# OrangeSodahub/InfGen

Measured on AMD Instinct MI355X. Metric: agent-steps/sec (closed-loop rollout), higher is better.
Workload: dtype f32

## Files before the change

### include/infgen_hip.h

```cpp
#ifndef INFGEN_HIP_H_
#define INFGEN_HIP_H_

#include <stdint.h>

#ifdef __cplusplus
extern "C" {
#endif

#define INFGEN_MAX_LAYERS 8

enum {
  INFGEN_Q_ATTN_PACK_SIZE = 0,
  INFGEN_Q_FOURIER_PACK_SIZE_N2 = 1,
  INFGEN_Q_FOURIER_PACK_SIZE_N3 = 2,
  INFGEN_Q_FOURIER_PACK_SIZE_N4 = 3,
  INFGEN_Q_TILE_ROWS = 4,
  INFGEN_Q_EDGE_ATTN_CAP = 5,
  INFGEN_Q_MAX_AGENTS = 6,
  INFGEN_Q_ABI_VERSION = 7,
  INFGEN_Q_SIZEOF_ROLLOUT = 8,
  INFGEN_Q_ATTN_SPLIT_ROWS = 9,
  INFGEN_Q_HEADS_SAMPLE_K = 10,
};
int infgen_layout_query(int what);
// ... 103 lines not shown
                    float* Q, float* U, float* K, float* V, void* stream);
int infgen_edge_attn(int rows, const float* Q, const float* U, const float* Ksrc, const float* Vsrc,
                     const int* off, const int* cnt, const int* src, const float* rhat,
                     float* AGG, float* Z, float* SIG, void* stream);
int infgen_edge_attn_fused(int rows, const float* Q, const float* pack, const float* Ksrc, const float* Vsrc,
                           const int* off, const int* cnt, const int* src, const float* rhat,
                           float* AGG, void* stream);
int infgen_fourier_embed_r24(const float* raw, int n_dims, const int* count_dev, int e_cap, const float* pack, void* out, void* stream);
int infgen_edge_attn_fused_r24(int rows, const float* Q, const float* pack, const float* Ksrc, const float* Vsrc,
                               const int* off, const int* cnt, const int* src, const void* rhat24, float* AGG, void* stream);
int infgen_set_rhat_format(int format);
int infgen_set_edge_kernel(int kernel);
int infgen_set_edge_fuse(int mode);
int infgen_get_options(InfgenOptions* out);
int infgen_thread_options(const InfgenOptions* o);
int infgen_get_effective_options(InfgenOptions* out);
int infgen_edge_fused_occupancy(void);
int infgen_debug_stream_read(const float* p, unsigned long long n_bytes, int width, float* out, void* stream);
int infgen_set_edge_loop(int variant);
int infgen_set_overlap(int mode);
int infgen_set_layers_p(int mode);
int infgen_layers_p_capacity(void);
int infgen_edge_attn_mode(int rows, const float* Q, const float* U, const float* Ksrc, const float* Vsrc,
                          const int* off, const int* cnt, const int* src, const float* rhat,
                          float* AGG, float* Z, float* SIG, int wide, void* stream);
int infgen_attn_post(float* X, int rows, const float* pack, const float* AGG, const float* Z, const float* SIG,
                     int has_pos, void* stream);
int infgen_attn_post_pre(float* X, int rows, const float* pack, const float* AGG, const float* Z, const float* SIG,
                         int has_pos, const float* next_pack, float* nQ, float* nU, float* nK, float* nV, void* stream);
int infgen_heads(const float* X, int rows, const float* tok_pack, const float* st_pack, int token_size,
                 float* logits, int* next_token, int* next_state, void* stream);
int infgen_heads_logprob(const float* X, int rows, const float* tok_pack, const float* st_pack, int token_size,
                         float* logits, int* next_token, int* next_state, float* token_logprob, void* stream);
int infgen_token_logprob(const float* logits, int rows, int n, const int* token, float* out, void* stream);
int infgen_heads_sample(const float* X, int rows, const float* tok_pack, const float* st_pack, int token_size, int k,
                        const float* uniform, float* logits, int* next_token, int* next_state, float* token_logprob,
                        float* sample_logprob, void* stream);
int infgen_heads_sample_ex(const float* X, int rows, const float* tok_pack, const float* st_pack, int token_size, int k,
                           const float* uniform, const InfgenSampling* sampling, float* logits, int* next_token, int* next_state,
                           float* token_logprob, float* sample_logprob, void* stream);
int infgen_heads_sample_mask(const float* X, int rows, const float* tok_pack, const float* st_pack, int token_size, int k,
                             const float* uniform, const InfgenSampling* sampling, const uint32_t* mask_bits, int mask_n_sets,
                             const int* mask_row, const int* mask_type, const int* type, float* logits,
                             int* next_token, int* next_state, float* token_logprob, float* sample_logprob, void* stream);
int infgen_heads_sample_fused(int attn_mode, int rows, int k);
int infgen_heads_logprob_fused(int attn_mode, int rows);
int infgen_map_token_head(const float* X, int ldx, const int* gather, int n, const float* pack, int token_size,
                          float* hidden, float* logits, long long* top_idx, void* stream);
int infgen_embedding_sum4(const float* tab0, const long long* idx0, int n0, const float* tab1, const long long* idx1, int n1,
                          const float* tab2, const long long* idx2, int n2, const float* tab3, const long long* idx3, int n3,
                          int rows, float* out, void* stream);
int infgen_map_graph(int S, int M_cap, const int* n_map, const float* pos, const float* orient, float radius,
                     int max_nbr, int* off, int* cnt, int* src, float* raw, int* total, int cap, void* stream);

int infgen_rollout_validate(const InfgenRollout* r);
int infgen_build_edges(const InfgenRollout* r, int c, int edgeless, void* stream);
int infgen_integrate(const InfgenRollout* r, int t, void* stream);
int infgen_raw_feature(const InfgenRollout* r, int col, void* stream);
int infgen_raw_feature_rows(const InfgenRollout* r, int col, const int* row_list, const int* row_mask, int n, void* stream);
int infgen_decode_layers(const InfgenRollout* r, int c, int edgeless, void* stream);
int infgen_decode_step(const InfgenRollout* r, int t, void* stream);
int infgen_rollout_run(const InfgenRollout* r, int t0, int t1, void* stream);
int infgen_command_rows(const InfgenRollout* r, int t, int kind, const int* cmd_token, const float* cmd_pose,
                        const unsigned char* cmd_mask, const float* shape, float* cmd_cost, void* stream);

int infgen_branch_scenes(const InfgenRollout* r, int t, const int* parent, int* n_bad, void* stream);
int infgen_resample_parents(const int* ancestor, int S0, int copies, int* parent, void* stream);

int infgen_snapshot_bytes(const InfgenRollout* r, int t, long long* bytes);
int infgen_snapshot_scenes(const InfgenRollout* r, int t, const int* slots, int n, void* snap, long long entry_stride, int* head,
                           int* n_bad, void* stream);
int infgen_restore_scenes(const InfgenRollout* r, int t, const int* index, const void* snap, long long entry_stride, const int* head,
                          int n, int* n_bad, void* stream);

int infgen_sample_topk(const float* logits, int rows, int n, int k, const float* uniform, int* token, void* stream);
int infgen_sample_topk_logprob(const float* logits, int rows, int n, int k, const float* uniform, int* token,
                               float* sample_logprob, void* stream);
int infgen_sample_topk_ex(const float* logits, int rows, int n, int k, const float* uniform, const InfgenSampling* sampling,
                          int* token, float* sample_logprob, int* nucleus, void* stream);
int infgen_sample_topk_mask(const float* logits, int rows, int n, int k, const float* uniform, const InfgenSampling* sampling,
                            const uint32_t* mask_bits, int mask_n_sets, const int* mask_row, const int* mask_type, const int* type,
                            int* token, float* sample_logprob, int* nucleus, void* stream);
int infgen_token_mask_create(const uint32_t* mask_bits, int mask_n_sets, const int* mask_row, const int* mask_type, const int* type);
int infgen_token_mask_destroy(int handle);

int infgen_collision_end_poses(const float* vocab, int token_size, float* end_pose, void* stream);
int infgen_collision_mask(const float* pos, const float* head, const int* state, const int* n_agents, const int* first_new,
                          const int* type, const float* shape, int S, int A_cap, int T, int c, const float* end_pose, int token_size,
                          int predict, float margin, const uint32_t* mask_bits, int mask_n_sets, const int* mask_row,
                          const int* mask_type, uint32_t* out_bits, int* out_count, void* stream);
int infgen_token_mask_collision(int handle, uint32_t* dyn_bits, const int* identity_row, const float* shape, const float* end_pose,
                                int predict, float margin, int* count);

int infgen_road_records_from_map(const float* map_pos, const float* map_orient, const long long* map_type, const long long* map_tok,
                                 const int* n_map, int S0, int M_cap, const float* map_vocab, int n_token, int detail, float* records,
                                 int rec_cap, int* n_records, void* stream);
int infgen_road_records_from_segments(const float* segments, const int* n_segments, int S0, int E, float* records, int rec_cap,
                                      int* n_records, void* stream);
int infgen_road_paths(const float* end_pose, int token_size, float* paths, void* stream);
int infgen_road_mask(const float* pos, const float* head, const int* state, const int* n_agents, const int* first_new, const int* type,
                     const float* shape, int S, int A_cap, int T, int c, const float* end_pose, const float* paths, int token_size,
                     const float* records, const int* n_records, int rec_cap, int copies, int sweep, float margin, const int* types,
                     const uint32_t* mask_bits, int mask_n_sets, const int* mask_row, const int* mask_type, uint32_t* out_bits,
                     int* out_count, void* stream);
int infgen_token_mask_road(int handle, uint32_t* road_bits, const int* identity_row, const float* shape, const float* end_pose,
                           const float* paths, const float* records, const int* n_records, int rec_cap, int copies, int sweep,
// ... 190 lines not shown
```

### infgen_amd/csrc/api.hip

```cpp
#include <cstdio>
#include <cstring>
#include <cstdlib>
#include <cmath>
#include <string>
#include <vector>
#include <atomic>
#include <mutex>
#include <unordered_map>
#include "kernels.h"
#include "../../include/infgen_hip.h"

using namespace ig;

static thread_local std::string g_err;

static int fail(const char* where, const char* what) {
  g_err = std::string(where) + ": " + what;
  return -1;
}
static int check_launch(const char* where) {
  hipError_t e = hipGetLastError();
  if (e != hipSuccess) return fail(where, hipGetErrorString(e));
  return 0;
}
// ... 651 lines not shown
}

extern "C" int infgen_edge_attn_fused(int rows, const float* Q, const float* pack, const float* Ksrc, const float* Vsrc,
                                      const int* off, const int* cnt, const int* src, const float* rhat,
                                      float* AGG, void* stream) {
  return edge_fused_launch(rows, Q, pack, Ksrc, Vsrc, EdgeSet{off, cnt, src, rhat}, AGG, 0, 0, stream);
}

extern "C" int infgen_fourier_embed_r24(const float* raw, int n, const int* count_dev, int e_cap, const float* pack, void* out,
                                        void* stream) {
  return fourier_embed_impl(raw, n, count_dev, e_cap, pack, nullptr, 0, static_cast<float*>(out), 128, 1, 1, stream);
}

extern "C" int infgen_edge_attn_fused_r24(int rows, const float* Q, const float* pack, const float* Ksrc, const float* Vsrc,
                                          const int* off, const int* cnt, const int* src, const void* rhat24,
                                          float* AGG, void* stream) {
  return edge_fused_launch(rows, Q, pack, Ksrc, Vsrc, EdgeSet{off, cnt, src, static_cast<const float*>(rhat24)}, AGG, 0, 0, stream, 1);
}

extern "C" int infgen_edge_attn(int rows, const float* Q, const float* U, const float* Ksrc, const float* Vsrc,
                                const int* off, const int* cnt, const int* src, const float* rhat,
                                float* AGG, float* Z, float* SIG, void* stream) {
  return edge_attn_impl(rows, Q, U, Ksrc, Vsrc, off, cnt, src, rhat, AGG, Z, SIG, rows <= 256 ? 1 : 0, stream);
}

extern "C" int infgen_edge_attn_mode(int rows, const float* Q, const float* U, const float* Ksrc, const float* Vsrc,
                                     const int* off, const int* cnt, const int* src, const float* rhat,
                                     float* AGG, float* Z, float* SIG, int wide, void* stream) {
  return edge_attn_impl(rows, Q, U, Ksrc, Vsrc, off, cnt, src, rhat, AGG, Z, SIG, wide, stream);
}

static int attn_post_fused(float* X, int rows, const float* pack, const float* AGG, const float* Z, const float* SIG,
                           int has_pos, const float* next_pack, float* nQ, float* nU, float* nK, float* nV, void* stream) {
  if (rows <= 0) return 0;
  { ProfScope _ps(INFGEN_KID_ATTN_POST, stream, attn_post_macs(rows, has_pos, next_pack, nQ, nU, nK, nV));
    if (attn_kind(rows)) {
      launch_attn_h(AttnHArgs{X, rows, pack, AGG, Z, SIG, has_pos, next_pack, 0, nQ, nU, nK, nV}, stream);
    } else {
      AttnPostArgs a{X, rows, pack, AGG, Z, SIG, has_pos, next_pack, nQ, nU, nK, nV};
      hipLaunchKernelGGL(k_attn_post, dim3(ceil_div(rows, TR)), dim3(NT), 0, (hipStream_t)stream, a);
    } }
  return check_launch("infgen_attn_post");
}

extern "C" int infgen_attn_post(float* X, int rows, const float* pack, const float* AGG, const float* Z,
                                const float* SIG, int has_pos, void* stream) {
  return attn_post_fused(X, rows, pack, AGG, Z, SIG, has_pos, nullptr, nullptr, nullptr, nullptr, nullptr, stream);
}

extern "C" int infgen_attn_post_pre(float* X, int rows, const float* pack, const float* AGG, const float* Z,
                                    const float* SIG, int has_pos, const float* next_pack, float* nQ, float* nU,
                                    float* nK, float* nV, void* stream) {
  return attn_post_fused(X, rows, pack, AGG, Z, SIG, has_pos, next_pack, nQ, nU, nK, nV, stream);
}

extern "C" int infgen_match_agent_tokens(const unsigned char* valid, const float* pos, const float* heading, const float* shape,
                                        const int* type, const float* tok, long long tok_agent_stride, int A, int T, int shift,
                                        int n_token, int* token_index, float* token_contour, void* stream) {
  if (A <= 0) return 0;
  if (shift <= 0 || T <= shift) return fail("infgen_match_agent_tokens", "need 0 < shift < T");
  if (n_token <= 0 || n_token > 2048) return fail("infgen_match_agent_tokens", "n_token must be in 1..2048");
  MatchTokensArgs a{valid, pos, heading, shape, type, tok, tok_agent_stride, A, T, shift, n_token, token_index, token_contour};
  hipLaunchKernelGGL(k_match_tokens, dim3(A), dim3(256), 0, (hipStream_t)stream, a);
  return check_launch("infgen_match_agent_tokens");
}

extern "C" int infgen_tokenize_agent(unsigned char* valid, float* pos, float* heading, float* velocity, const int* type,
                                    const float* tok, const float* shape_in, float* shape_out, float* wl_work, int A, int T,
                                    int shift, int current_step, int n_token, int invalid_state, int valid_state,
                                    int enter_state, int exit_state, int predict_state, int* token_index,
                                    float* token_contour, int* state_idx, float* token_pos, float* token_heading,
                                    unsigned char* token_valid, unsigned char* raw_token_valid, void* stream) {
  if (A <= 0) return 0;
  if (shift <= 0 || T <= shift || current_step < shift || current_step >= T)
    return fail("infgen_tokenize_agent", "need 0 < shift <= current_step < T");
  if (n_token <= 0 || n_token > 2048) return fail("infgen_tokenize_agent", "n_token must be in 1..2048");
  TokenizeArgs t{valid, pos, heading, velocity, type, wl_work, shape_in, shape_out, A, T, shift, current_step,
                 invalid_state, valid_state, enter_state, exit_state, predict_state, token_index, token_contour,
                 state_idx, token_pos, token_heading, token_valid, raw_token_valid};
  hipLaunchKernelGGL(k_tokenize_prep, dim3((A + 63) / 64), dim3(64), 0, (hipStream_t)stream, t);
  MatchTokensArgs m{valid, pos, heading, wl_work, type, tok, 0, A, T, shift, n_token, token_index, token_contour};
  hipLaunchKernelGGL(k_match_tokens, dim3(A), dim3(256), 0, (hipStream_t)stream, m);
  hipLaunchKernelGGL(k_tokenize_state, dim3((A + 63) / 64), dim3(64), 0, (hipStream_t)stream, t);
  return check_launch("infgen_tokenize_agent");
}

extern "C" int infgen_fetch_enterings(const float* token_pos, const float* token_heading, const int* state_idx,
                                     const int* agent_ptr, const int* av_index, int B, int max_agents, int T,
                                     const float* grid_xy, int grid_size, float radius, float angle_interval,
                                     int enter_state, int invalid_state, int* grid_token_idx, float* grid_offset_xy,
                                     int* heading_token_idx, int* sort_indices, unsigned char* inrange_mask,
                                     unsigned char* bos_mask, float* pos_xy, float* heading_theta, const float* pt_pos,
                                     int pt_stride, const int* pt_ptr, int M, int* pt_grid_token_idx, void* stream) {
  if (B <= 0 || T <= 0) return 0;
  if (max_agents > 2048) return fail("infgen_fetch_enterings", "more than 2048 agents in a scene");
  if (grid_size <= 0) return fail("infgen_fetch_enterings", "empty grid");
  EnteringsArgs a{token_pos, token_heading, state_idx, agent_ptr, av_index, B, T, grid_xy, grid_size, radius, angle_interval,
                  enter_state, invalid_state, grid_token_idx, grid_offset_xy, heading_token_idx, sort_indices, inrange_mask,
                  bos_mask, pos_xy, heading_theta, pt_pos, pt_stride, pt_ptr, M, pt_grid_token_idx};
  hipLaunchKernelGGL(k_fetch_enterings, dim3(B * T), dim3(256), 0, (hipStream_t)stream, a);
  if (pt_grid_token_idx && M > 0) {
    const long long waves = (long long)T * M;
    hipLaunchKernelGGL(k_pt_grid_cells, dim3((unsigned)((waves + 3) / 4)), dim3(256), 0, (hipStream_t)stream, a);
  }
  return check_launch("infgen_fetch_enterings");
}
// ... 1777 lines not shown
```

### infgen_amd/csrc/attn_h.hip

```cpp
#include <type_traits>
#include "kernels.h"
#include "layout.h"
#include "tile.cuh"
#include "split.cuh"
#include "attn_h.cuh"

namespace ig {

template <int WAVES, int TERMS>
__global__ __launch_bounds__(64 * WAVES, WAVES == 4 ? 2 : 1) void k_attn_h(AttnHArgs a) {
  constexpr int NTH = 64 * WAVES, TILE = 16 * WAVES;
  constexpr int XRING = WAVES == 4 ? IG_AH_RING4 : IG_AH_RING8;
  __shared__ __attribute__((aligned(16))) unsigned short Wb[XRING][QUARTER];
  __shared__ __attribute__((aligned(16))) float Vt[VT_SIZE];
  __shared__ const unsigned short* seg_ptr[5];
  __shared__ int seg_n[5];
  const int ngroups = a.groups ? *a.n_groups : (a.rows + 15) / 16;
  const int ntiles = (ngroups + WAVES - 1) / WAVES;
  if ((int)blockIdx.x >= ntiles) return;
  const int tid = threadIdx.x;
  const int lane = tid & 63, w = tid >> 6;
  const int j = lane & 15, rg = lane >> 4;
  const float* P = a.pack;
  const float* NP = a.next_pack;
// ... 181 lines not shown
        if (need_u) {
          u32x4 Qh[4], Ql[4];
          const float cq = frags_scaled(q, Qh, Ql) * hdr[1];
          float* urow = valid ? a.nU + (size_t)row * (H * D) : nullptr;
          for (int hp = 0; hp < 4; ++hp) {
            const unsigned short* Wl = take();
#pragma unroll
            for (int hh = 0; hh < 2; ++hh) {
              u32x2 qh, ql;
#define IG_PICK(S) case S: qh = hh ? u32x2{Qh[S][2], Qh[S][3]} : u32x2{Qh[S][0], Qh[S][1]}; \
                           ql = hh ? u32x2{Ql[S][2], Ql[S][3]} : u32x2{Ql[S][0], Ql[S][1]}; break;
              switch (hp) { IG_PICK(0) IG_PICK(1) IG_PICK(2) default: IG_PICK(3) }
#undef IG_PICK
              const v4h vqh = __builtin_bit_cast(v4h, qh), vql = __builtin_bit_cast(v4h, ql);
#pragma unroll
              for (int ct = 0; ct < 8; ++ct) {
                const v4h ah = *reinterpret_cast<const v4h*>(Wl + ((hh * 8 + ct) * 2) * 256 + lane * 4);
                const v4h al = *reinterpret_cast<const v4h*>(Wl + ((hh * 8 + ct) * 2 + 1) * 256 + lane * 4);
                f32x4 acc = {0.f, 0.f, 0.f, 0.f};
                acc = __builtin_amdgcn_mfma_f32_16x16x16f16(ah, vqh, acc, 0, 0, 0);
                if constexpr (TERMS == 3) {
                  acc = __builtin_amdgcn_mfma_f32_16x16x16f16(ah, vql, acc, 0, 0, 0);
                  acc = __builtin_amdgcn_mfma_f32_16x16x16f16(al, vqh, acc, 0, 0, 0);
                }
                if (urow)
                  *reinterpret_cast<float4*>(urow + (2 * hp + hh) * D + 16 * ct + 4 * rg) =
                      make_float4(acc[0] * cq, acc[1] * cq, acc[2] * cq, acc[3] * cq);
              }
            }
          }
        }
      }
      if (need_kv) {
        f32x4 kk[8];
        zero_acc(kk);
        gemm_unit(kk, Bh, Bl);
        scale_bias(kk, inv_n * hdr[2], nullptr, rg);
        store_row(valid ? a.nK + (size_t)row * D : nullptr, kk, rg);
        zero_acc(kk);
        gemm_unit(kk, Bh, Bl);
        scale_bias(kk, inv_n * hdr[3], Vt + VT_N_BV, rg);
        store_row(valid && a.nV ? a.nV + (size_t)row * D : nullptr, kk, rg);
      }
    }
  }
}

#if !IG_BF16_OPERANDS
template __global__ void k_attn_h<4, 3>(AttnHArgs);
template __global__ void k_attn_h<8, 3>(AttnHArgs);
#endif
template __global__ void k_attn_h<4, 1>(AttnHArgs);

__global__ __launch_bounds__(1024) void k_active_groups(ActiveGroupsArgs a) {
  __shared__ int wave_cnt[16];
  __shared__ int base;
  const int total = (a.S * a.A_cap + 15) / 16;
  const int lane = threadIdx.x & 63, w = threadIdx.x >> 6;
  if (threadIdx.x == 0) base = 0;
  __syncthreads();
  for (int g0 = 0; g0 < total; g0 += 1024) {
    const int g = g0 + threadIdx.x;
    bool on = false;
    if (g < total) {
      const int r0 = 16 * g, r1 = min(16 * g + 15, a.S * a.A_cap - 1);
      const int s0 = r0 / a.A_cap, s1 = r1 / a.A_cap;
      on = (r0 - s0 * a.A_cap) < a.n_agents[s0] + a.margin;
      if (s1 != s0) on = on || a.n_agents[s1] + a.margin > 0;
    }
    const unsigned long long m = __ballot(on);
    if (lane == 0) wave_cnt[w] = __popcll(m);
    __syncthreads();
    int off = base;
    for (int k = 0; k < w; ++k) off += wave_cnt[k];
    if (on) a.groups[off + __popcll(m & ((1ull << lane) - 1))] = g;
    __syncthreads();
    if (threadIdx.x == 0) { int t = 0; for (int k = 0; k < 16; ++k) t += wave_cnt[k]; base += t; }
    __syncthreads();
  }
  if (threadIdx.x == 0) *a.n_groups = base;
}

}
```

### infgen_amd/csrc/attn_h_b16.hip

```cpp
#define IG_BF16_OPERANDS 1
#define k_attn_h k_attn_h_b16
#define k_active_groups k_active_groups_b16_unused
#include "attn_h.hip"
```

### infgen_amd/csrc/kernels.h

```cpp
#pragma once
#include <type_traits>
#include "tile.cuh"
#include "layout.h"
#include "../../include/infgen_hip.h"

namespace ig {

struct LinearArgs {
  const float* X; int ldx; const int* gather;
  int rows; int K; int Kp;
  const float* Wp; int Np; const float* bias; int N;
  const float* pre_g; const float* pre_b;
  const float* post_g; const float* post_b; int relu;
  float* Y; int ldy;
};

constexpr int LINEAR_MULTI_MAX = 6;
struct LinearMultiArgs { LinearArgs d[LINEAR_MULTI_MAX]; };

struct FourierArgs {
  const float* raw;
  int n;
  const int* count_dev;
  int e_cap;
// ... 68 lines not shown
  int rows;
  const float* Q;
  const float* pack;
  const float* Ksrc; const float* Vsrc;
  EdgeSet es;
  float* AGG;
  const int* groups; const int* n_groups;
  int dbg;
  int tiles_per_scene;
  int kv_once;
  int n_virtual;
  unsigned* dbgbuf;
  WarmArgs warm;
};

constexpr int LP_MAX_LAYERS = 8;
struct LayersPArgs {
  int rows, A_cap, num_layers;
  int xcd_order;
  int row0;
  int rows_per_wg;
  float* X;
  const float* attn_t[LP_MAX_LAYERS]; const float* attn_m[LP_MAX_LAYERS]; const float* attn_a[LP_MAX_LAYERS];
  float* ringK[LP_MAX_LAYERS]; float* ringV[LP_MAX_LAYERS];
  size_t slot_off;
  const float* mapK[LP_MAX_LAYERS]; const float* mapV[LP_MAX_LAYERS];
  float* Ka[2]; float* Va[2];
  EdgeSet et, em, ea;
  int* sync;
  unsigned spin_limit;
  unsigned long long* trace;
};

struct AttnPostArgs {
  float* X; int rows;
  const float* pack;
  const float* AGG; const float* Z; const float* SIG;
  int has_pos;
  const float* next_pack;
  float* nQ; float* nU; float* nK; float* nV;
};

struct AttnHArgs {
  float* X; int rows;
  const float* pack;
  const float* AGG; const float* Z; const float* SIG;
  int has_pos;
  const float* next_pack;
  int next_src_ln;
  float* nQ; float* nU; float* nK; float* nV;
  const int* groups; const int* n_groups;
  int dbg;
  WarmArgs warm;
};

struct ActiveGroupsArgs { const int* n_agents; int S, A_cap, margin; int* groups; int* n_groups; };

struct NearestArgs {
  const float* cx; const float* cy; const float* length; const float* width; const float* heading;
  const unsigned char* valid;
  int B, N, T, n_eval;
  float rounding;
  float* work;
  float* out;
};

struct KinematicArgs {
  const float* x; const float* y; const float* z; const float* heading;
  int n, T; float dt;
  float* speed; float* accel; float* yaw_rate; float* yaw_accel;
};
struct TtcArgs {
  const float* cx; const float* cy; const float* length; const float* width; const float* heading; const float* speed;
  const unsigned char* valid;
  const int* eval_idx;
  int B, N, T, n_eval;
  float* out;
};

struct TokenizeArgs {
  unsigned char* valid; float* pos; float* heading; float* velocity;
  const int* type; float* wl;
  const float* shape_in; float* shape_out;
  int A, T, shift, current_step;
  int invalid_state, valid_state, enter_state, exit_state, predict_state;
  int* token_index; const float* token_contour;
  int* state_idx; float* token_pos; float* token_heading;
  unsigned char* token_valid; unsigned char* raw_token_valid;
};

struct EnteringsArgs {
  const float* token_pos; const float* token_heading; const int* state_idx;
  const int* agent_ptr; const int* av_index;
  int B, T; const float* grid_xy; int grid_size;
  float radius, angle_interval; int enter_state, invalid_state;
  int* grid_token_idx; float* grid_offset_xy; int* heading_token_idx; int* sort_indices;
  unsigned char* inrange_mask; unsigned char* bos_mask; float* pos_xy; float* heading_theta;
  const float* pt_pos; int pt_stride; const int* pt_ptr; int M; int* pt_grid_token_idx;
};

struct RoadEdgeArgs {
  const float* cx; const float* cy; const float* cz; const float* length; const float* width; const float* height;
  const float* heading; const unsigned char* valid; const int* eval_idx;
  const float* poly; const unsigned char* cyclic; const int* poly_off;
  int B, N, T, n_eval, L; float z_stretch;
  float* out;
// ... 421 lines not shown
  int copies, sweep; float margin; int types[3]; float dt;
  float* out; long long out_stride;
  unsigned char* out_row;
};
__global__ void k_step_score(ScoreArgs a);

struct TokenLogprobArgs {
  const float* logits; int rows; int n;
  const int* token;
  float* out;
};

constexpr int MAP_GRAPH_C = 8;
struct MapGraphArgs {
  int S, M_cap; const int* n_map;
  const float* pos; const float* orient; float radius; int max_nbr;
  EdgeBuf e;
  int lds_tokens;
};

template <int W> __global__ void k_stream_read(const float* p, size_t n_floats, float* out);
__global__ void k_linear(LinearArgs a);
__global__ void k_linear_multi(LinearMultiArgs m);
__global__ void k_fourier(FourierArgs a);
template <int TERMS> __global__ void k_fourier_h(FourierArgs a);
template <int TERMS> __global__ void k_fourier_h_multi(FourierMultiArgs m);
template <int TERMS> __global__ void k_fourier_h12(FourierArgs a);
template <int TERMS> __global__ void k_fourier_h12_multi(FourierMultiArgs m);
constexpr int FH12_NT = 768, FH12_TILE = 192;
__global__ void k_match_tokens(MatchTokensArgs a);
template <int TERMS> __global__ void k_mlpemb_h(MlpEmbHArgs a);
__global__ void k_box_corners(NearestArgs a);
__global__ void k_nearest_distance(NearestArgs a);
__global__ void k_kinematic(KinematicArgs a);
__global__ void k_ttc(TtcArgs a);
__global__ void k_placement(PlacementArgs a);
__global__ void k_window_loglik(WindowLoglikArgs a);
__global__ void k_bundle_field(BundleScoreArgs a);
__global__ void k_bundle_meta(BundleScoreArgs a);
__global__ void k_road_edge(RoadEdgeArgs a);
template <int TERMS, bool LP = false, int KS = 0, bool MK = false> __global__ void k_heads_h(ArgsFor<HeadsArgs, MK> a);
template <int TERMS> __global__ void k_map_head_h(MapHeadArgs a);
template <int TERMS> __global__ void k_map_head_h_b16(MapHeadArgs a);
__global__ void k_map_topk(MapHeadArgs a);
__global__ void k_match_map_tokens(MatchMapArgs a);
__global__ void k_command_rows(CommandRowsArgs a);
__global__ void k_tokenize_prep(TokenizeArgs a);
__global__ void k_fetch_enterings(EnteringsArgs a);
__global__ void k_pt_grid_cells(EnteringsArgs a);
__global__ void k_tokenize_state(TokenizeArgs a);
__global__ void k_active_groups(ActiveGroupsArgs a);
template <int WAVES, int TERMS> __global__ void k_attn_h(AttnHArgs a);
template <int WAVES, int TERMS> __global__ void k_attn_h_b16(AttnHArgs a);
template <int TERMS> __global__ void k_attn_hs_b16(AttnHArgs a);
template <int TERMS> __global__ void k_mlpemb_h_b16(MlpEmbHArgs a);
template <int TERMS, bool LP, int KS, bool MK> __global__ void k_heads_h_b16(ArgsFor<HeadsArgs, MK> a);
template <int TERMS> __global__ void k_fourier_h_b16(FourierArgs a);
template <int TERMS> __global__ void k_fourier_h_multi_b16(FourierMultiArgs m);
template <int TERMS> __global__ void k_attn_hs(AttnHArgs a);
__global__ void k_attn_pre(AttnPreArgs a);
__global__ void k_edge_attn(EdgeAttnArgs a);
template <int G> __global__ void k_edge_fused3(EdgeFusedArgs a);
template <int G, bool R24, int HALVES, int WAVES> __global__ void k_edge_fused(EdgeFusedArgs a);
template <bool R24, int ROWS> __global__ void k_layers_p(LayersPArgs a);
__global__ void k_edge_attn_wide(EdgeAttnArgs a);
__global__ void k_attn_post(AttnPostArgs a);
template <bool MK> __global__ void k_heads(ArgsFor<HeadsArgs, MK> a);
template <int BT> __global__ void k_build_edges(BuildEdgesArgs a);
template <int BT> __global__ void k_integrate(IntegrateArgs a);
__global__ void k_rawfeat_prep(RawFeatArgs a);
__global__ void k_scatter_rows(const float* src, const int* row_list, const int* row_mask, int n, float* dst);
__global__ void k_scatter_rows2(const float* src0, const float* src1, const int* row_list, const int* row_mask, int n, float* dst0,
                                float* dst1);
__global__ void k_note_riders(const int* new_row, const int* inserted, int n, int* prev_row, int* prev_mask, int* pend_row,
                              int* pend_mask);
struct EmbedSum4Args {
  const float* tab[4]; const long long* idx[4]; int n[4];
  int rows; float* out;
};
__global__ void k_embedding_sum4(EmbedSum4Args a);
__global__ void k_gather_rows(const float* src, const int* row_list, const int* row_mask, int n, int limit, float* dst);
__global__ void k_insert_cat(InsertCatArgs a);
__global__ void k_map_graph(MapGraphArgs a);
__global__ void k_point_edges(PointEdgesArgs a);
__global__ void k_occupancy(OccupancyArgs a);
__global__ void k_occupancy_embed(OccEmbedArgs a);
template <bool kGrid> __global__ void k_insert_decide(InsertDecideArgs a);
template <bool kHeadToken, bool kOffset> __global__ void k_insert_finalize(InsertFinalizeArgs a);
template <bool MK> __global__ void k_sample_topk(ArgsFor<SampleArgs, MK> a);
__global__ void k_token_logprob(TokenLogprobArgs a);
__global__ void k_layernorm(const float* X, int rows, const float* g, const float* b, float* Y);
__global__ void k_radius_edges(RadiusEdgesArgs a);
__global__ void k_motion_features(MotionFeatArgs a);

constexpr int MAX_SCENE_AGENTS = 1024;
constexpr int PACK_MAX_KEYS = 32;
struct PackRowsArgs {
  const char* src[PACK_MAX_KEYS]; char* dst[PACK_MAX_KEYS]; long long src_stride[PACK_MAX_KEYS];
  const int* counts[PACK_MAX_KEYS]; int count_stride[PACK_MAX_KEYS]; int row_bytes[PACK_MAX_KEYS];
  int n_keys, n_scenes, scene0, scene_step;
};
__global__ void k_ingest_batch(InfgenBatchIngest a);
__global__ void k_pack_rows(PackRowsArgs a);

constexpr int VM_MAX_PARTIALS = 1024;
constexpr int GO_MAX_CELLS = 16384;
// ... 41 lines not shown
```

### infgen_amd/engine.py

```python
from __future__ import annotations

import ctypes as C
import hashlib
import os
from typing import Dict, List, Mapping, Optional, Sequence

import numpy as np
import torch

from . import _lib, constraints, logprob, packing, scene_setup
from .scene_setup import EVAL_SHAPE, INVALID_SHAPE
from .synth import INVALID, VALID, ENTER, EXIT, AGENT_SHAPE, RolloutConfig

D = 128
SEED_TYPE = 3


def _round_up(x: int, m: int) -> int:
    return (x + m - 1) // m * m


class LazyOut(dict):
    __slots__ = ('_lazy',)

# ... 271 lines not shown
                       'infgen_map_token_head')
        return logits, top

    def mlp_embedding(self, x, pack, k0, out=None):
        k0p, o1, o2, o3 = packing.mlp_embedding_offsets(k0)
        h = self.linear(x, pack, o1, 128, k0, bias_off=o1 + k0p * 128, post_ln_off=o1 + k0p * 128 + 128, relu=True)
        h = self.linear(h, pack, o2, 128, 128, bias_off=o2 + 16384, post_ln_off=o2 + 16384 + 128, relu=True)
        return self.linear(h, pack, o3, 128, 128, bias_off=o3 + 16384, out=out)

    def mlp_layer(self, x, pack, k0, n_out, out=None):
        k0p = _round_up(k0, 8)
        o_b0 = k0p * 128
        h = self.linear(x, pack, 0, 128, k0, bias_off=o_b0, post_ln_off=o_b0 + 128, relu=True)
        o_w3 = o_b0 + 3 * 128
        return self.linear(h, pack, o_w3, n_out, 128, bias_off=o_w3 + 128 * _round_up(n_out, 32), out=out)

    def mlp_layers(self, x, packs_nout):
        rows, n = x.shape[0], len(packs_nout)
        hid = torch.empty(n, rows, 128, device=self.device, dtype=torch.float32)
        outs = [torch.empty(rows, no, device=self.device, dtype=torch.float32) for _, no in packs_nout]
        d1, d2 = (_lib.LinearDesc * n)(), (_lib.LinearDesc * n)()
        o_b0, o_w3 = 128 * 128, 128 * 128 + 3 * 128
        for i, (pack, no) in enumerate(packs_nout):
            base = pack.data_ptr()
            a = d1[i]
            a.X, a.ldx, a.gather, a.rows, a.K = x.data_ptr(), x.stride(0), None, rows, 128
            a.Wp, a.Np, a.bias, a.N = base, 128, base + 4 * o_b0, 128
            a.pre_g = a.pre_b = None
            a.post_g, a.post_b, a.relu = base + 4 * (o_b0 + 128), base + 4 * (o_b0 + 256), 1
            a.Y, a.ldy = hid[i].data_ptr(), 128
            b = d2[i]
            npad = _round_up(no, 32)
            b.X, b.ldx, b.gather, b.rows, b.K = hid[i].data_ptr(), 128, None, rows, 128
            b.Wp, b.Np, b.bias, b.N = base + 4 * o_w3, npad, base + 4 * (o_w3 + 128 * npad), no
            b.pre_g = b.pre_b = b.post_g = b.post_b = None
            b.relu = 0
            b.Y, b.ldy = outs[i].data_ptr(), outs[i].stride(0)
        _lib.check(self.lib.infgen_linear_multi(d1, n, self.stream), 'infgen_linear_multi')
        _lib.check(self.lib.infgen_linear_multi(d2, n, self.stream), 'infgen_linear_multi')
        return outs

    def fourier(self, raw, n, pack, out, count_dev=None, rows=None, cat=None, normalize=False):
        rows = raw.shape[0] if rows is None else rows
        _lib.check(self.lib.infgen_fourier_embed(_lib.ptr(raw), n, _lib.ptr(count_dev), rows, _lib.ptr(pack),
                                                 _lib.ptr(cat), cat.stride(0) if cat is not None else 0,
                                                 out.data_ptr(), out.stride(0), int(normalize), self.stream),
                   'infgen_fourier_embed')
        return out

    def attn_pre(self, x, pack, use_src_ln=False, q=None, u=None, k=None, v=None, rows=None):
        rows = x.shape[0] if rows is None else rows
        _lib.check(self.lib.infgen_attn_pre(_lib.ptr(x), rows, _lib.ptr(pack), int(use_src_ln), _lib.ptr(q),
                                            _lib.ptr(u), _lib.ptr(k), _lib.ptr(v), self.stream), 'infgen_attn_pre')

    def edge_attn(self, rows, q, u, ksrc, vsrc, off, cnt, src, rhat, agg, z, sig, wide=None):
        args = (rows, _lib.ptr(q), _lib.ptr(u), _lib.ptr(ksrc), _lib.ptr(vsrc), _lib.ptr(off), _lib.ptr(cnt),
                _lib.ptr(src), _lib.ptr(rhat), _lib.ptr(agg), _lib.ptr(z), _lib.ptr(sig))
        if wide == 'fused':
            _lib.check(self.lib.infgen_edge_attn_fused(rows, _lib.ptr(q), _lib.ptr(u), *args[3:10], self.stream),
                       'infgen_edge_attn_fused')
        elif wide is None:
            _lib.check(self.lib.infgen_edge_attn(*args, self.stream), 'infgen_edge_attn')
        else:
            _lib.check(self.lib.infgen_edge_attn_mode(*args, int(wide), self.stream), 'infgen_edge_attn_mode')

    def attn_post(self, x, pack, agg, z, sig, has_pos=True, rows=None):
        rows = x.shape[0] if rows is None else rows
        _lib.check(self.lib.infgen_attn_post(_lib.ptr(x), rows, _lib.ptr(pack), _lib.ptr(agg), _lib.ptr(z),
                                             _lib.ptr(sig), int(has_pos), self.stream), 'infgen_attn_post')

    def attn_post_pre(self, x, pack, agg, z, sig, next_pack, has_pos=True, q=None, u=None, k=None, v=None):
        _lib.check(self.lib.infgen_attn_post_pre(_lib.ptr(x), x.shape[0], _lib.ptr(pack), _lib.ptr(agg), _lib.ptr(z),
                                                 _lib.ptr(sig), int(has_pos), _lib.ptr(next_pack), _lib.ptr(q), _lib.ptr(u),
                                                 _lib.ptr(k), _lib.ptr(v), self.stream), 'infgen_attn_post_pre')

    def attention_layer(self, x, pack, off, cnt, src, rhat, x_src=None, scratch=None, wide=None):
        rows = x.shape[0]
        dev = self.device
        sc = scratch if scratch is not None else {}
        q = sc.get('Q', torch.empty(rows, D, device=dev))
        u = sc.get('U', torch.empty(rows, 8 * D, device=dev))
        agg = sc.get('AGG', torch.empty(rows, D, device=dev))
        z = sc.get('Z', torch.empty(rows, 8 * D, device=dev))
        sig = sc.get('SIG', torch.empty(rows, 8, device=dev))
        fused = wide == 'fused'
        if x_src is None:
            k = torch.empty(rows, D, device=dev)
            v = torch.empty(rows, D, device=dev)
            self.attn_pre(x, pack, q=q, u=None if fused else u, k=k, v=v)
        else:
            k = torch.empty(x_src.shape[0], D, device=dev)
            v = torch.empty(x_src.shape[0], D, device=dev)
            self.attn_pre(x_src, pack, use_src_ln=True, k=k, v=v)
            self.attn_pre(x, pack, q=q, u=None if fused else u)
        self.edge_attn(rows, q, pack if fused else u, k, v, off, cnt, src, rhat, agg, z, sig, wide=wide)
        self.attn_post(x, pack, agg, z, sig, has_pos=rhat is not None and not fused)
        return x


def _edge_index(data):
    try:
        return data[('pt_token', 'to', 'map_polygon')]['edge_index']
    except (KeyError, TypeError):
        return data['pt_token__to__map_polygon']['edge_index']


# ... 924 lines not shown
        self.reset()
        if self._coll is not None:
            self._coll['shape'].copy_(self._shape10.reshape(rows, 3))
        if self.stay_on_road is not None:
            self._road['shape'].copy_(self._shape10.reshape(rows, 3))
            if self._road_dirty:
                self._road_build()
        if self.step_scores is not None:
            if self.stay_on_road is None:
                self._score_boxes().copy_(self._shape10.reshape(rows, 3))
            if self._road_dirty:
                self._road_build()
        if self.cat_agent is None:
            self.cat_agent = torch.empty(rows, D, device=dev)
        shp = ops.mlp_embedding(self._shape10.reshape(rows, 3), w.shape_emb, 3)
        torch.add(w.type_a_emb[self.atype.reshape(-1).long()], shp, out=self.cat_agent)

        if self._x_pt_override is not None:
            return self._prologue_with_given_map()
        S0 = self.S0
        mrows = S0 * M_cap
        mtok, mtype, mpl, mlight = self._map_cat
        if self.x_pt is None:
            self.x_pt = torch.empty(mrows, D, device=dev)
        mt = tabs['map_tab']
        _lib.check(self.lib.infgen_embedding_sum4(_lib.ptr(mt), _lib.ptr(mtok), mt.shape[0], _lib.ptr(w.type_pt_emb), _lib.ptr(mtype),
                                                  w.type_pt_emb.shape[0], _lib.ptr(w.polygon_type_emb), _lib.ptr(mpl),
                                                  w.polygon_type_emb.shape[0], _lib.ptr(w.light_pl_emb), _lib.ptr(mlight),
                                                  w.light_pl_emb.shape[0], mrows, _lib.ptr(self.x_pt), ops.stream),
                   'infgen_embedding_sum4')
        x_pt = self.x_pt
        K = 100
        if self._mg is None:
            cap = mrows * self._map_nbr_cap
            self._mg = dict(off=torch.zeros(mrows, device=dev, dtype=torch.int32),
                            cnt=torch.zeros(mrows, device=dev, dtype=torch.int32),
                            src=torch.zeros(cap, device=dev, dtype=torch.int32), raw=torch.zeros(cap, 4, device=dev),
                            rhat=torch.empty(cap, D, device=dev), total=torch.zeros(1, device=dev, dtype=torch.int32),
                            cap=cap, K=torch.empty(mrows, D, device=dev), V=torch.empty(mrows, D, device=dev),
                            Q=torch.empty(mrows, D, device=dev), AGG=torch.empty(mrows, D, device=dev))
        g = self._mg
        _lib.check(self.lib.infgen_map_graph(S0, M_cap, _lib.ptr(self.n_map), _lib.ptr(self.map_pos),
                                             _lib.ptr(self.map_orient), float(cfg.pl2pl_radius), K, _lib.ptr(g['off']),
                                             _lib.ptr(g['cnt']), _lib.ptr(g['src']), _lib.ptr(g['raw']),
                                             _lib.ptr(g['total']), g['cap'], ops.stream), 'infgen_map_graph')
        if not self._mg_checked:
            tot = int(g['total'].item())
            if tot > g['cap']:
                self._map_nbr_cap = (tot + mrows - 1) // mrows + 4
                self._mg = None
                return self._prologue(map_only=map_only)
            self._mg_checked = True
        fused = bool(self.flags['map_fuse'])
        eo = self._effective_options()
        r24 = fused and eo.rhat_format == 1 and eo.fourier_mode != 0
        if r24:
            _lib.check(self.lib.infgen_fourier_embed_r24(_lib.ptr(g['raw']), 3, _lib.ptr(g['total']), g['cap'], _lib.ptr(w.four_pt),
                                                         g['rhat'].data_ptr(), ops.stream), 'infgen_fourier_embed_r24')
        else:
            ops.fourier(g['raw'], 3, w.four_pt, g['rhat'], count_dev=g['total'], rows=g['cap'], normalize=True)
        for i in range(cfg.num_map_layers):
            if not fused:
                if 'U' not in g:
                    g.update(U=torch.empty(mrows, 8 * D, device=dev), Z=torch.empty(mrows, 8 * D, device=dev),
                             SIG=torch.empty(mrows, 8, device=dev))
                ops.attn_pre(x_pt, w.attn_pt[i], q=g['Q'], u=g['U'], k=g['K'], v=g['V'])
                ops.edge_attn(mrows, g['Q'], g['U'], g['K'], g['V'], g['off'], g['cnt'], g['src'], g['rhat'],
                              g['AGG'], g['Z'], g['SIG'])
                ops.attn_post(x_pt, w.attn_pt[i], g['AGG'], g['Z'], g['SIG'])
                continue
            if i == 0:
                ops.attn_pre(x_pt, w.attn_pt[0], q=g['Q'], k=g['K'], v=g['V'])
            if r24:
                _lib.check(self.lib.infgen_edge_attn_fused_r24(mrows, _lib.ptr(g['Q']), _lib.ptr(w.attn_pt[i]), _lib.ptr(g['K']),
                                                               _lib.ptr(g['V']), _lib.ptr(g['off']), _lib.ptr(g['cnt']),
                                                               _lib.ptr(g['src']), g['rhat'].data_ptr(), _lib.ptr(g['AGG']),
                                                               ops.stream), 'infgen_edge_attn_fused_r24')
            else:
                ops.edge_attn(mrows, g['Q'], w.attn_pt[i], g['K'], g['V'], g['off'], g['cnt'], g['src'], g['rhat'],
                              g['AGG'], None, None, wide='fused')
            if i + 1 < cfg.num_map_layers:
                ops.attn_post_pre(x_pt, w.attn_pt[i], g['AGG'], None, None, w.attn_pt[i + 1], has_pos=False,
                                  q=g['Q'], k=g['K'], v=g['V'])
            else:
                ops.attn_post(x_pt, w.attn_pt[i], g['AGG'], None, None, has_pos=False)
        if map_only:
            return
        self._finish_prologue()

    def map_token_head(self, rows: torch.Tensor):
        with _lib.thread_options(self._effective_options()):
            return self.ops.map_token_head(self.x_pt, rows.to(self.device, torch.int32).contiguous(), self.w.map_head)

    def _prologue_with_given_map(self):
        S0, M_cap, dev = self.S0, self.M_cap, self.device
        if self.x_pt is None:
            self.x_pt = torch.zeros(S0 * M_cap, D, device=dev)
        assert len(self._x_pt_override) == S0, 'one x_pt per distinct scene'
        for s, xp in enumerate(self._x_pt_override):
            M = self.hosts[s * self.copies]['M']
            self.x_pt[s * M_cap:s * M_cap + M] = xp.detach().to(dev, torch.float32)
        self._finish_prologue()

    def _finish_prologue(self):
        ops, w, cfg = self.ops, self.w, self.cfg
        x_pt = self.x_pt
        for i in range(cfg.num_agent_layers):
            ops.attn_pre(x_pt, w.attn_m[i], use_src_ln=True, k=self.mapK[i], v=self.mapV[i])

        if self.insertion:
            self._alloc_insertion()
            for i in range(3):
                ops.attn_pre(x_pt, w.attn_pt2sa[i], use_src_ln=True, k=self.ins['mapK'][i], v=self.ins['mapV'][i])
        if self._ctx is None:
            self._build_ctx()
        self._refresh_opts()
        self._decoded_rows.zero_()
        st = ops.stream
        _lib.check(self.lib.infgen_raw_feature(C.byref(self._ctx), 0, st), 'raw_feature(0)')
        _lib.check(self.lib.infgen_decode_layers(C.byref(self._ctx), 0, 1, st), 'decode_layers(0)')
        _lib.check(self.lib.infgen_raw_feature(C.byref(self._ctx), 1, st), 'raw_feature(1)')
        self._prologue_done = True

    def rollout(self):
        self._bc_host = None
        self._end_session()
        if (self._graph_all and not self.insertion and self._x_pt_override is None and self._mg_checked and self._init is not None
                and self._ctx is not None and not _lib.prof_active()):
            self._rollout_graph()
            return
        self.prologue()
        self.run()

    def _rollout_graph(self):
        cur = torch.cuda.current_stream(self.device)
        if getattr(self, '_gstream', None) is None:
            self._gstream = torch.cuda.Stream(device=self.device)
        gs = self._gstream
        gs.wait_stream(cur)
        with torch.cuda.stream(gs):
            self._refresh_opts(groups=True)
            snap = bytes(self._ctx.opts)[:_lib.OPTIONS_VALUE_BYTES] + bytes([self._ctx.four_t_dt is not None])
            if self._wgraph is not None and snap != self._wgraph_opts:
                self._wgraph = None
            if self._wgraph is None:
                g = torch.cuda.CUDAGraph()
                with torch.cuda.graph(g, stream=gs):
                    self.prologue()
                    self.run()
                self._wgraph, self._wgraph_opts = g, snap
            self._wgraph.replay()
            self._prologue_done = True
        cur.wait_stream(gs)

    def _alloc_insertion(self):
        if self.ins is not None:
            for k in ('n_new', 'active', 'inserted'):
                self.ins[k].zero_()
            self.ins['shape_all'].fill_(INVALID_SHAPE)
            self.ins['first_new'].fill_(self.A_cap)
            self.ins['inserted_rows'] = [[] for _ in range(self.S)]
            if self.seed_out is not None:
                for v in self.seed_out.values():
                    v.zero_()
            return
        dev, S, rows, A_cap, M_cap, G = self.device, self.S, self.rows, self.A_cap, self.M_cap, self.G
# ... 752 lines not shown
```

Baseline: 29.84 million.

## Fuse per-layer map K/V projections into one multi-layer kernel and native map encode

Adds a kernel that loads each map row once, computes the shared layernorm statistics, and writes K/V projections for up to nine attention layers in a single launch. Before this, each layer ran its own attn_pre. It also moves the fused map-encoder loop (fourier embed, attn_pre, edge attention, post/pre) from Python into a single C entry point to cut host-side dispatch overhead. The cost is another kernel variant with a heavier shared-memory footprint, and a fallback path for other attention modes.

New measurement: 29.96 million (median of 2 runs). Within noise of the previous version (+0.4%).

```diff
diff --git a/include/infgen_hip.h b/include/infgen_hip.h
--- a/include/infgen_hip.h
+++ b/include/infgen_hip.h
@@ -179,6 +179,10 @@
                           int rows, float* out, void* stream);
 int infgen_map_graph(int S, int M_cap, const int* n_map, const float* pos, const float* orient, float radius,
                      int max_nbr, int* off, int* cnt, int* src, float* raw, int* total, int cap, void* stream);
+int infgen_map_kv_multi(const float* X, int rows, int n, const float* const* packs, float* const* K, float* const* V, void* stream);
+int infgen_map_encode(int rows, const int* off, const int* cnt, const int* src, const float* raw, const int* total, int cap,
+                      void* rhat, const float* four_pack, float* x_pt, float* Q, float* K, float* V, float* AGG,
+                      const float* const* packs, int num_map_layers, void* stream);
 
 int infgen_rollout_validate(const InfgenRollout* r);
 int infgen_build_edges(const InfgenRollout* r, int c, int edgeless, void* stream);
diff --git a/infgen_amd/csrc/api.hip b/infgen_amd/csrc/api.hip
--- a/infgen_amd/csrc/api.hip
+++ b/infgen_amd/csrc/api.hip
@@ -727,6 +727,62 @@
                                     const float* SIG, int has_pos, const float* next_pack, float* nQ, float* nU,
                                     float* nK, float* nV, void* stream) {
   return attn_post_fused(X, rows, pack, AGG, Z, SIG, has_pos, next_pack, nQ, nU, nK, nV, stream);
+}
+
+extern "C" int infgen_map_kv_multi(const float* X, int rows, int n, const float* const* packs, float* const* K, float* const* V,
+                                   void* stream) {
+  if (rows <= 0 || n == 0) return 0;
+  if (n < 0 || n > ATTN_KV_MULTI_MAX) return fail("infgen_map_kv_multi", "n must be in 0..9");
+  if (!X || !packs || !K || !V) return fail("infgen_map_kv_multi", "null pointer");
+  for (int i = 0; i < n; ++i)
+    if (!packs[i] || !K[i] || !V[i]) return fail("infgen_map_kv_multi", "every layer needs its pack, K and V");
+  { ProfScope _ps(INFGEN_KID_ATTN_PRE, stream, (double)n * attn_pre_macs(rows, nullptr, nullptr, K[0], V[0]));
+    if (attn_kind(rows) == 1 && knob::attn_waves != 8) {
+      AttnKVMultiArgs a{X, rows, n, {}, {}, {}, knob::qs_dbg};
+      for (int i = 0; i < n; ++i) { a.pack[i] = packs[i]; a.K[i] = K[i]; a.V[i] = V[i]; }
+      t_warm = WarmArgs{};
+      hipLaunchKernelGGL(by_terms(k_attn_kv_multi<3>, k_attn_kv_multi_b16<1>, k_attn_kv_multi<1>), dim3(grid64(rows)), dim3(256), 0,
+                         (hipStream_t)stream, a);
+    } else {
+      for (int i = 0; i < n; ++i) {
+        if (attn_kind(rows)) {
+          launch_attn_h(AttnHArgs{const_cast<float*>(X), rows, nullptr, nullptr, nullptr, nullptr, 0, packs[i], 1, nullptr, nullptr, K[i], V[i]}, stream);
+        } else {
+          AttnPreArgs p{X, rows, packs[i], 1, nullptr, nullptr, K[i], V[i]};
+          hipLaunchKernelGGL(k_attn_pre, dim3(ceil_div(rows, TR)), dim3(NT), 0, (hipStream_t)stream, p);
+        }
+      }
+    } }
+  return check_launch("infgen_map_kv_multi");
+}
+
+struct MapEncodeArgs {
+  int rows; EdgeSet es; const float* raw; const int* total; int cap; const float* four_pack;
+  float* x_pt; float* Q; float* K; float* V; float* AGG; const float* const* packs; int num_map_layers;
+};
+static int map_encode_impl(const MapEncodeArgs& m, void* stream) {
+  const bool r24 = O().rhat_format == 1 && O().fourier_mode != 0;
+  float* rhat = const_cast<float*>(m.es.rhat);
+  RET_IF(fourier_embed_impl(m.raw, 3, m.total, m.cap, m.four_pack, nullptr, 0, rhat, 128, 1, r24 ? 1 : 0, stream));
+  RET_IF(infgen_attn_pre(m.x_pt, m.rows, m.packs[0], 0, m.Q, nullptr, m.K, m.V, stream));
+  for (int i = 0; i < m.num_map_layers; ++i) {
+    RET_IF(edge_fused_launch(m.rows, m.Q, m.packs[i], m.K, m.V, m.es, m.AGG, 0, 0, stream, r24 ? 1 : 0));
+    const float* next = i + 1 < m.num_map_layers ? m.packs[i + 1] : nullptr;
+    RET_IF(attn_post_fused(m.x_pt, m.rows, m.packs[i], m.AGG, nullptr, nullptr, 0, next, next ? m.Q : nullptr, nullptr,
+                           next ? m.K : nullptr, next ? m.V : nullptr, stream));
+  }
+  return 0;
+}
+extern "C" int infgen_map_encode(int rows, const int* off, const int* cnt, const int* src, const float* raw, const int* total, int cap,
+                                 void* rhat, const float* four_pack, float* x_pt, float* Q, float* K, float* V, float* AGG,
+                                 const float* const* packs, int num_map_layers, void* stream) {
+  if (rows <= 0) return 0;
+  if (num_map_layers < 1 || num_map_layers > INFGEN_MAX_LAYERS) return fail("infgen_map_encode", "num_map_layers must be in 1..8");
+  if (!off || !cnt || !src || !raw || !total || !rhat || !four_pack || !x_pt || !Q || !K || !V || !AGG || !packs)
+    return fail("infgen_map_encode", "null pointer");
+  for (int i = 0; i < num_map_layers; ++i) if (!packs[i]) return fail("infgen_map_encode", "every layer needs its pack");
+  return map_encode_impl(MapEncodeArgs{rows, EdgeSet{off, cnt, src, static_cast<const float*>(rhat)}, raw, total, cap, four_pack,
+                                       x_pt, Q, K, V, AGG, packs, num_map_layers}, stream);
 }
 
 extern "C" int infgen_match_agent_tokens(const unsigned char* valid, const float* pos, const float* heading, const float* shape,
diff --git a/infgen_amd/csrc/attn_h.hip b/infgen_amd/csrc/attn_h.hip
--- a/infgen_amd/csrc/attn_h.hip
+++ b/infgen_amd/csrc/attn_h.hip
@@ -257,6 +257,78 @@
 #endif
 template __global__ void k_attn_h<4, 1>(AttnHArgs);
 
+template <int TERMS>
+__global__ __launch_bounds__(256, 2) void k_attn_kv_multi(AttnKVMultiArgs a) {
+  constexpr int NTH = 256, WAVES = 4;
+  constexpr int KV_G = 0, KV_B = 128, KV_BV = 256, KV_HDR = 384, KV_VT = 400;
+  __shared__ __attribute__((aligned(16))) unsigned short Wb[IG_AH_RING4][QUARTER];
+  __shared__ __attribute__((aligned(16))) float Vt[ATTN_KV_MULTI_MAX * KV_VT];
+  __shared__ const unsigned short* seg_ptr[ATTN_KV_MULTI_MAX];
+  __shared__ int seg_n[ATTN_KV_MULTI_MAX];
+  const int ngroups = (a.rows + 15) / 16;
+  const int ntiles = (ngroups + WAVES - 1) / WAVES;
+  if ((int)blockIdx.x >= ntiles) return;
+  const int tid = threadIdx.x;
+  const int lane = tid & 63, w = tid >> 6;
+  const int j = lane & 15, rg = lane >> 4;
+  if (tid < a.n) {
+    seg_ptr[tid] = reinterpret_cast<const unsigned short*>(a.pack[tid] + AH_PRE) + 8 * QUARTER;
+    seg_n[tid] = 8;
+  }
+  for (int l = 0; l < a.n; ++l) {
+    const float* NP = a.pack[l];
+    float* vt = Vt + l * KV_VT;
+    for (int i = tid; i < 128; i += NTH) {
+      vt[KV_G + i] = NP[AL_LN_SRC_G + i]; vt[KV_B + i] = NP[AL_LN_SRC_B + i]; vt[KV_BV + i] = NP[AL_BV + i];
+    }
+    if (tid < 16) vt[KV_HDR + tid] = NP[AH_HDR + tid];
+  }
+  __syncthreads();
+  QuarterStream<NTH, IG_AH_RING4> qs;
+  qs.dbg = a.dbg;
+  qs.init(seg_ptr, seg_n, a.n, (ntiles - (int)blockIdx.x + (int)gridDim.x - 1) / (int)gridDim.x, Wb, tid);
+  auto gemm_unit = [&](f32x4 (&acc)[8], const u32x4 (&Bh)[4], const u32x4 (&Bl)[4]) {
+#pragma unroll
+    for (int s = 0; s < 4; ++s) gemm_quarter<TERMS>(acc, qs.take(), Bh[s], Bl[s], lane);
+  };
+
+  for (int tile = blockIdx.x; tile < ntiles; tile += gridDim.x) {
+    const int grp = tile * WAVES + w;
+    const int row = grp * 16 + j;
+    const bool valid = grp < ngroups && row < a.rows;
+    const int rowc = valid ? row : a.rows - 1;
+    f32x4 x[8];
+    load_row_nc(x, a.X + (size_t)rowc * D, rg);
+    const float rstd = ln_stats(x);
+    for (int l = 0; l < a.n; ++l) {
+      const float* vt = Vt + l * KV_VT;
+      const float* hdr = vt + KV_HDR;
+      f32x4 xn[8];
+#pragma unroll
+      for (int t = 0; t < 8; ++t) xn[t] = x[t];
+      LnTab tb;
+      ln_fetch(tb, vt + KV_G, vt + KV_B, rg);
+      ln_apply_tab<false>(xn, rstd, tb);
+      u32x4 Bh[4], Bl[4];
+      const float inv_n = frags_scaled(xn, Bh, Bl);
+      f32x4 kk[8];
+      zero_acc(kk);
+      gemm_unit(kk, Bh, Bl);
+      scale_bias(kk, inv_n * hdr[2], nullptr, rg);
+      store_row(valid ? a.K[l] + (size_t)row * D : nullptr, kk, rg);
+      zero_acc(kk);
+      gemm_unit(kk, Bh, Bl);
+      scale_bias(kk, inv_n * hdr[3], vt + KV_BV, rg);
+      store_row(valid ? a.V[l] + (size_t)row * D : nullptr, kk, rg);
+    }
+  }
+}
+
+#if !IG_BF16_OPERANDS
+template __global__ void k_attn_kv_multi<3>(AttnKVMultiArgs);
+#endif
+template __global__ void k_attn_kv_multi<1>(AttnKVMultiArgs);
+
 __global__ __launch_bounds__(1024) void k_active_groups(ActiveGroupsArgs a) {
   __shared__ int wave_cnt[16];
   __shared__ int base;
diff --git a/infgen_amd/csrc/attn_h_b16.hip b/infgen_amd/csrc/attn_h_b16.hip
--- a/infgen_amd/csrc/attn_h_b16.hip
+++ b/infgen_amd/csrc/attn_h_b16.hip
@@ -1,4 +1,5 @@
 #define IG_BF16_OPERANDS 1
 #define k_attn_h k_attn_h_b16
+#define k_attn_kv_multi k_attn_kv_multi_b16
 #define k_active_groups k_active_groups_b16_unused
 #include "attn_h.hip"
diff --git a/infgen_amd/csrc/kernels.h b/infgen_amd/csrc/kernels.h
--- a/infgen_amd/csrc/kernels.h
+++ b/infgen_amd/csrc/kernels.h
@@ -144,6 +144,15 @@
   const int* groups; const int* n_groups;
   int dbg;
   WarmArgs warm;
+};
+
+constexpr int ATTN_KV_MULTI_MAX = 9;
+struct AttnKVMultiArgs {
+  const float* X; int rows;
+  int n;
+  const float* pack[ATTN_KV_MULTI_MAX];
+  float* K[ATTN_KV_MULTI_MAX]; float* V[ATTN_KV_MULTI_MAX];
+  int dbg;
 };
 
 struct ActiveGroupsArgs { const int* n_agents; int S, A_cap, margin; int* groups; int* n_groups; };
@@ -671,6 +680,8 @@
 __global__ void k_active_groups(ActiveGroupsArgs a);
 template <int WAVES, int TERMS> __global__ void k_attn_h(AttnHArgs a);
 template <int WAVES, int TERMS> __global__ void k_attn_h_b16(AttnHArgs a);
+template <int TERMS> __global__ void k_attn_kv_multi(AttnKVMultiArgs a);
+template <int TERMS> __global__ void k_attn_kv_multi_b16(AttnKVMultiArgs a);
 template <int TERMS> __global__ void k_attn_hs_b16(AttnHArgs a);
 template <int TERMS> __global__ void k_mlpemb_h_b16(MlpEmbHArgs a);
 template <int TERMS, bool LP, int KS, bool MK> __global__ void k_heads_h_b16(ArgsFor<HeadsArgs, MK> a);
diff --git a/infgen_amd/engine.py b/infgen_amd/engine.py
--- a/infgen_amd/engine.py
+++ b/infgen_amd/engine.py
@@ -347,6 +347,13 @@
         rows = x.shape[0] if rows is None else rows
         _lib.check(self.lib.infgen_attn_pre(_lib.ptr(x), rows, _lib.ptr(pack), int(use_src_ln), _lib.ptr(q),
                                             _lib.ptr(u), _lib.ptr(k), _lib.ptr(v), self.stream), 'infgen_attn_pre')
+
+    def map_kv_multi(self, x, sets):
+        for s0 in range(0, len(sets), 9):
+            part = sets[s0:s0 + 9]
+            packs, ks, vs = ((C.c_void_p * len(part))(*[_lib.ptr(t[j]) for t in part]) for j in range(3))
+            _lib.check(self.lib.infgen_map_kv_multi(_lib.ptr(x), x.shape[0], len(part), packs, ks, vs, self.stream),
+                       'infgen_map_kv_multi')
 
     def edge_attn(self, rows, q, u, ksrc, vsrc, off, cnt, src, rhat, agg, z, sig, wide=None):
         args = (rows, _lib.ptr(q), _lib.ptr(u), _lib.ptr(ksrc), _lib.ptr(vsrc), _lib.ptr(off), _lib.ptr(cnt),
@@ -1377,38 +1384,22 @@
                 return self._prologue(map_only=map_only)
             self._mg_checked = True
         fused = bool(self.flags['map_fuse'])
-        eo = self._effective_options()
-        r24 = fused and eo.rhat_format == 1 and eo.fourier_mode != 0
-        if r24:
-            _lib.check(self.lib.infgen_fourier_embed_r24(_lib.ptr(g['raw']), 3, _lib.ptr(g['total']), g['cap'], _lib.ptr(w.four_pt),
-                                                         g['rhat'].data_ptr(), ops.stream), 'infgen_fourier_embed_r24')
+        if fused:
+            packs = (C.c_void_p * cfg.num_map_layers)(*[w.attn_pt[i].data_ptr() for i in range(cfg.num_map_layers)])
+            _lib.check(self.lib.infgen_map_encode(mrows, _lib.ptr(g['off']), _lib.ptr(g['cnt']), _lib.ptr(g['src']), _lib.ptr(g['raw']),
+                                                  _lib.ptr(g['total']), g['cap'], g['rhat'].data_ptr(), _lib.ptr(w.four_pt),
+                                                  _lib.ptr(x_pt), _lib.ptr(g['Q']), _lib.ptr(g['K']), _lib.ptr(g['V']),
+                                                  _lib.ptr(g['AGG']), packs, cfg.num_map_layers, ops.stream), 'infgen_map_encode')
         else:
             ops.fourier(g['raw'], 3, w.four_pt, g['rhat'], count_dev=g['total'], rows=g['cap'], normalize=True)
-        for i in range(cfg.num_map_layers):
-            if not fused:
-                if 'U' not in g:
-                    g.update(U=torch.empty(mrows, 8 * D, device=dev), Z=torch.empty(mrows, 8 * D, device=dev),
-                             SIG=torch.empty(mrows, 8, device=dev))
+            if 'U' not in g:
+                g.update(U=torch.empty(mrows, 8 * D, device=dev), Z=torch.empty(mrows, 8 * D, device=dev),
+                         SIG=torch.empty(mrows, 8, device=dev))
+            for i in range(cfg.num_map_layers):
                 ops.attn_pre(x_pt, w.attn_pt[i], q=g['Q'], u=g['U'], k=g['K'], v=g['V'])
                 ops.edge_attn(mrows, g['Q'], g['U'], g['K'], g['V'], g['off'], g['cnt'], g['src'], g['rhat'],
                               g['AGG'], g['Z'], g['SIG'])
                 ops.attn_post(x_pt, w.attn_pt[i], g['AGG'], g['Z'], g['SIG'])
-                continue
-            if i == 0:
-                ops.attn_pre(x_pt, w.attn_pt[0], q=g['Q'], k=g['K'], v=g['V'])
-            if r24:
-                _lib.check(self.lib.infgen_edge_attn_fused_r24(mrows, _lib.ptr(g['Q']), _lib.ptr(w.attn_pt[i]), _lib.ptr(g['K']),
-                                                               _lib.ptr(g['V']), _lib.ptr(g['off']), _lib.ptr(g['cnt']),
-                                                               _lib.ptr(g['src']), g['rhat'].data_ptr(), _lib.ptr(g['AGG']),
-                                                               ops.stream), 'infgen_edge_attn_fused_r24')
-            else:
-                ops.edge_attn(mrows, g['Q'], w.attn_pt[i], g['K'], g['V'], g['off'], g['cnt'], g['src'], g['rhat'],
-                              g['AGG'], None, None, wide='fused')
-            if i + 1 < cfg.num_map_layers:
-                ops.attn_post_pre(x_pt, w.attn_pt[i], g['AGG'], None, None, w.attn_pt[i + 1], has_pos=False,
-                                  q=g['Q'], k=g['K'], v=g['V'])
-            else:
-                ops.attn_post(x_pt, w.attn_pt[i], g['AGG'], None, None, has_pos=False)
         if map_only:
             return
         self._finish_prologue()
@@ -1430,13 +1421,11 @@
     def _finish_prologue(self):
         ops, w, cfg = self.ops, self.w, self.cfg
         x_pt = self.x_pt
-        for i in range(cfg.num_agent_layers):
-            ops.attn_pre(x_pt, w.attn_m[i], use_src_ln=True, k=self.mapK[i], v=self.mapV[i])
-
+        sets = [(w.attn_m[i], self.mapK[i], self.mapV[i]) for i in range(cfg.num_agent_layers)]
         if self.insertion:
             self._alloc_insertion()
-            for i in range(3):
-                ops.attn_pre(x_pt, w.attn_pt2sa[i], use_src_ln=True, k=self.ins['mapK'][i], v=self.ins['mapV'][i])
+            sets += [(w.attn_pt2sa[i], self.ins['mapK'][i], self.ins['mapV'][i]) for i in range(3)]
+        ops.map_kv_multi(x_pt, sets)
         if self._ctx is None:
             self._build_ctx()
         self._refresh_opts()
```
